# TAdeJong/pyGPA

Hardware: AMD Instinct MI355X
Metric: Mpixels/s displacement-field extraction (3 peaks, 4096^2 img) + achieved HBM GB/s (higher is better)
Workload: dtype f32; 1 GPU; 4096x4096 synthetic hex moire, 3 Bragg peaks x 16 k-vectors, sigma=10, weighted DCT-PCG unwrap kmax=10, image resident in HBM, u downloaded to pinned host memory inside the step (BASELINE.json configs[2]); x_planes=12, d2h_of_u=included, overlapped with the next step (copy stream), images_in_flight=1

## Files before the change

### pygpa_amd/csrc/gpa_api.hip

```cpp
#include "gpa_plan.h"

static thread_local std::string g_err;
int gpa_fail(int code, const std::string& msg) {
  g_err = msg;
  return code;
}
namespace gpa {
static const char* const kOptNames[OPT_COUNT] = {
    "PBS_FULLBAND", "SERIAL_UNWRAP", "NO_WORKER", "NO_KSPLIT", "NO_COMPACT", "NO_SHARED",
    "NO_PAIR", "TRI_SMALL", "TRI_Q", "NO_MR", "MR_FORCE_BLUESTEIN", "NO_ROWPQ", "COLSOLVE", "NO_LAT",
    "F32_EPS_FLOOR", "COLSTREAM_CHUNK", "NO_ROWHALF", "PAIR_MAXSIDE", "ROWHALF_MINLG", "NO_PQDCT",
    "NO_REORDER", "NO_RAW", "NO_TILEFUSE", "NO_ROWPERS", "NO_LFTILE", "LF_ALL_ROUNDS", "DFT_ENGINE", "GAUSS_FFT_MINR", "NO_GAUSS2D", "NO_DFT_HALF", "F32_STALL", "PBS_LDS_PAD", "NO_SHARED_PHASES", "PA_STAG", "PA_STAG_TICKS", "PA_ROT", "LF_STACK_BYTES", "NO_YSPEC"};
static OptVal g_opts[OPT_COUNT];
static std::once_flag g_opts_once;
static void opt_assign(OptVal& o, const char* value) {
  o.set = value != nullptr;
  o.num = value ? atof(value) : 0.0;
  memset(o.str, 0, sizeof(o.str));
  if (value) strncpy(o.str, value, sizeof(o.str) - 1);
}
static void opts_from_env() {
  for (int k = 0; k < OPT_COUNT; ++k) opt_assign(g_opts[k], getenv((std::string("GPA_") + kOptNames[k]).c_str()));
}
const OptVal& opt(OptKey k) {
  std::call_once(g_opts_once, opts_from_env);
  return g_opts[k];
}
}

Axis make_axis(int n) {
  Axis a;
  a.n = n;
  int lg = 0;
  while ((1 << lg) < n) ++lg;
  if ((1 << lg) == n) {
    a.padded = false;
  } else {
    lg = 0;
    while ((1 << lg) < 2 * n - 1) ++lg;
    a.padded = true;
  }
  if (lg < 6) {
    lg = 6;
    a.padded = ((1 << lg) != n);
  }
// ... 149 lines not shown
  p->serial_unwrap = opt_set(OPT_SERIAL_UNWRAP);
  p->use_worker = !opt_set(OPT_NO_WORKER);
  p->no_ksplit = opt_set(OPT_NO_KSPLIT);
  p->no_compact = opt_set(OPT_NO_COMPACT);
  p->use_shared = !opt_set(OPT_NO_SHARED);
  const int maxlg = dtype == GPA_F32 ? 14 : 13;
  if (n0 > 65536 || n1 > 65536) {
    fail(GPA_ERR_ARG, "gpa_plan_create: axis longer than 65536");
    delete p;
    return nullptr;
  }
  p->spectral_only = p->ax0.lg > maxlg || p->ax1.lg > maxlg;
  auto unwrap_axis_ok = [&](const Axis& a) { return a.lg <= maxlg || (a.lg == 14 && a.n == 16384); };
  p->no_unwrap = !(unwrap_axis_ok(p->ax0) && unwrap_axis_ok(p->ax1));
  if (plan_build(p) != GPA_OK) {
    std::string keep = g_err;
    gpa_plan_destroy(p);
    g_err = keep;
    return nullptr;
  }
  return p;
}

void gpa_plan_destroy(gpa_plan* p) {
  if (!p) return;
  hipSetDevice(p->device);
  delete p->worker;
  p->worker = nullptr;
  if (p->stream) hipStreamSynchronize(p->stream);
  void* bufs[] = {p->tw0, p->tw1, p->Hx, p->Hy, p->Tbuf, p->tb.cxb, p->tb.sx, p->tb.wxw, p->tb.wxr, p->tb.cyb, p->tb.sy, p->tb.wyw, p->tb.wyr, p->tb.planeof, p->d_pw,
                  p->tb.dx, p->tb.dy, p->d_kl, p->d_kr, p->d_image, p->d_mean, p->d_tile_mean, p->d_scratch,
                  p->d_lockin, p->d_kidx, p->d_dudx, p->d_dudy, p->d_wnorm, p->d_u, p->d_kmat, p->d_sf, p->d_grad, p->d_grads, p->d_absw, p->d_aux0, p->d_aux1,
                  p->sh.Gb, p->sh.psi, p->sh.dyc, p->sh.gtab, p->sh.desc, p->sh.order, p->d_taps, p->tw1s,
                  p->sh.pre, p->sh.rot16, p->d_wys, p->d_shifts, p->d_ystep, p->ys.Yhat, p->ys.strips, p->d_ys_pairs};
  for (void* b : bufs)
    if (b) hipFree(b);
  unwrap_workspace_destroy(&p->uw);
  unwrap_workspace_destroy(&p->uw2);
  if (p->uwb_images) unwrap_workspace_destroy(&p->uwb);
  if (p->have_uwp) unwrap_workspace_destroy(&p->uwp);
  if (p->d_wnorm_b) (void)hipFree(p->d_wnorm_b);
  if (p->h_iters_b) (void)hipHostFree(p->h_iters_b);
  for (void* b : {p->bT, p->bL, p->bMean, (void*)p->bScratch})
    if (b) (void)hipFree(b);
  if (p->stream2) { hipStreamSynchronize(p->stream2); hipStreamDestroy(p->stream2); }
  if (p->ev_fork) hipEventDestroy(p->ev_fork);
  if (p->ev_join) hipEventDestroy(p->ev_join);
  if (p->ev_x) hipEventDestroy(p->ev_x);
  if (p->d_tsum_part) (void)hipFree(p->d_tsum_part);
  warp_ws_free(&p->warp);
  ucell_ws_free(&p->ucell);
  dft_axis_destroy(&p->bx0);
  dft_axis_destroy(&p->bx1);
  dft_work_free(&p->dftw);
  for (auto& ax : p->gft)
    for (auto& g : ax) {
      if (g.H) (void)hipFree(g.H);
      if (g.tw) (void)hipFree(g.tw);
    }
  if (p->d_pertab) (void)hipFree(p->d_pertab);
  if (p->d_peakws) (void)hipFree(p->d_peakws);
  if (p->d_peaksmooth) (void)hipFree(p->d_peaksmooth);
  if (p->h_k) hipHostFree(p->h_k);
  if (p->h_iters) hipHostFree(p->h_iters);
  if (p->kprof) {
    for (int i = 0; i < p->kprof->npool; ++i) hipEventDestroy(p->kprof->pool[i]);
    delete p->kprof;
// ... 83 lines not shown
```

### pygpa_amd/csrc/gpa_api_tables.hip

```cpp
#include "gpa_plan.h"

void host_fft_pow2(std::vector<std::complex<double>>& a, bool inverse) {
  const size_t n = a.size();
  int lg = 0;
  while ((size_t(1) << lg) < n) ++lg;
  for (size_t i = 0; i < n; ++i) {
    size_t r = 0;
    for (int b = 0; b < lg; ++b) r |= ((i >> b) & 1) << (lg - 1 - b);
    if (r > i) std::swap(a[i], a[r]);
  }
  for (size_t len = 2; len <= n; len <<= 1) {
    const double ang = (inverse ? 2 : -2) * M_PI / (double)len;
    for (size_t s = 0; s < n; s += len)
      for (size_t j = 0; j < len / 2; ++j) {
        std::complex<double> w(cos(ang * (double)j), sin(ang * (double)j));
        auto u = a[s + j], v = a[s + j + len / 2] * w;
        a[s + j] = u + v;
        a[s + j + len / 2] = u - v;
      }
  }
}

std::vector<double> gaussian_kspace(int n, double sigma) {
  std::vector<double> g(n);
// ... 122 lines not shown
          const int Epad = (E + 15) & ~15;
          if (sa.L != cur.L && p->tw1s_L != sa.L) {
            if (!p->tw1s) TRY(dmalloc(p, &p->tw1s, (size_t)8192 * p->csz));
            TRY(upload_twiddles(p, p->tw1s, sa.L));
            p->tw1s_L = sa.L;
          }
          p->ax1s = sa;
          if (!p->d_taps) TRY(dmalloc(p, (void**)&p->d_taps, 1025 * sizeof(double)));
          if (!p->sh.gtab) TRY(dmalloc(p, &p->sh.gtab, (2 * 256 + 16) * p->rsz));
          HIP_TRY(hipMemcpyAsync(p->d_taps, taps.data(), ((size_t)mmax + 1) * sizeof(double), hipMemcpyHostToDevice, p->stream));
          HIP_TRY(hipStreamSynchronize(p->stream));
          std::vector<double> gt((size_t)2 * Epad + 16, 0.0);
          for (int m = 1; m <= E; ++m) gt[m] = taps[m];
          TRY(upload_real_table(p, p->sh.gtab, gt));
          p->sh_etab = mmax;
          p->sh_E = E;
          p->sh_Epad = Epad;
          p->sh_sigma = sigma;
          p->sh_ok = true;
        }
      }
    }
  }
  p->sigma_cached = sigma;
  return GPA_OK;
}

int shared_prepare(gpa_plan* p, int P, int K) {
  p->sh_use = false;
  p->ys_use = false;
  const int B = P * K;
  if (!p->sh_ok || !p->use_shared || K < 2 || (int)p->staged_planeof.size() < B) return GPA_OK;
  const bool reorder = !opt_set(OPT_NO_REORDER);
  if (p->sh_built_epoch == p->sh_epoch && p->sh_built_K == K && p->sh_built_B == B && p->sh_built_reorder == reorder) {
    p->sh_use = p->sh_built_ok;
    return GPA_OK;
  }
  p->sh_built_reorder = reorder;
  p->sh_built_epoch = -1;
  p->sh_built_ok = false;
  std::vector<int> order((size_t)B);
  for (int pp = 0; pp < P; ++pp) {
    bool aliased = false;
    for (int a = 0; a < K && !aliased; ++a)
      for (int b2 = a + 1; b2 < K && !aliased; ++b2) {
        const double *ka = &p->staged_kl[2 * ((size_t)pp * K + a)], *kb = &p->staged_kl[2 * ((size_t)pp * K + b2)];
        const bool same = ka[0] == kb[0] && ka[1] == kb[1];
        aliased = !same && ka[0] - floor(ka[0]) == kb[0] - floor(kb[0]) && ka[1] - floor(ka[1]) == kb[1] - floor(kb[1]);
      }
    std::vector<double> d2((size_t)K), pmin;
    std::vector<int> pfirst;
    int nplanes = 0;
    for (int k = 0; k < K; ++k) nplanes = std::max(nplanes, p->staged_planeof[pp * K + k] + 1);
    pmin.assign((size_t)nplanes, 1e300);
    pfirst.assign((size_t)nplanes, K);
    for (int k = 0; k < K; ++k) {
      const size_t b = (size_t)pp * K + k;
      const double ex = p->staged_kl[2 * b] - p->staged_kr[2 * b], ey = p->staged_kl[2 * b + 1] - p->staged_kr[2 * b + 1];
      d2[k] = ex * ex + ey * ey;
      const int pl = p->staged_planeof[b];
      pmin[pl] = std::min(pmin[pl], d2[k]);
      pfirst[pl] = std::min(pfirst[pl], k);
    }
    std::vector<int> idx((size_t)K);
    for (int k = 0; k < K; ++k) idx[k] = k;
    if (reorder && !aliased)
      std::stable_sort(idx.begin(), idx.end(), [&](int a, int b2) {
        const int pa = p->staged_planeof[pp * K + a], pb = p->staged_planeof[pp * K + b2];
        if (pa != pb) return pmin[pa] != pmin[pb] ? pmin[pa] < pmin[pb] : pfirst[pa] < pfirst[pb];
        return d2[a] < d2[b2];
      });
// ... 66 lines not shown
    p->sh_psi_bytes = ps;
  }
  if (!p->sh.rot16) TRY(dmalloc(p, &p->sh.rot16, (size_t)p->max_peaks * 16 * p->csz));
  if (!p->d_wys) TRY(dmalloc(p, (void**)&p->d_wys, (size_t)p->max_batch * sizeof(double)));
  if (!p->d_shifts) TRY(dmalloc(p, (void**)&p->d_shifts, (size_t)p->max_peaks * sizeof(int)));
  HIP_TRY(hipMemcpyAsync(p->d_wys, wys.data(), (size_t)B * sizeof(double), hipMemcpyHostToDevice, p->stream));
  HIP_TRY(hipMemcpyAsync(p->d_shifts, shifts.data(), (size_t)P * sizeof(int), hipMemcpyHostToDevice, p->stream));
  {
    std::vector<double> ys((size_t)P);
    p->sh_one_kref = true;
    for (int pp = 0; pp < P; ++pp) {
      const double c = p->staged_kr[2 * ((size_t)pp * K) + 1] + (double)shifts[pp] / EEs;
      ys[pp] = 2.0 * M_PI * (c - rint(c));
      for (int k = 1; k < K; ++k)
        if (p->staged_kr[2 * ((size_t)pp * K + k) + 1] != p->staged_kr[2 * ((size_t)pp * K) + 1]) p->sh_one_kref = false;
    }
    if (!p->d_ystep) TRY(dmalloc(p, (void**)&p->d_ystep, (size_t)p->max_peaks * sizeof(double)));
    HIP_TRY(hipMemcpyAsync(p->d_ystep, ys.data(), (size_t)P * sizeof(double), hipMemcpyHostToDevice, p->stream));
    HIP_TRY(hipStreamSynchronize(p->stream));
  }
  if (!p->sh.dyc) TRY(dmalloc(p, &p->sh.dyc, (size_t)p->max_peaks * p->n1 * p->csz));
  if (!p->sh.desc) TRY(dmalloc(p, (void**)&p->sh.desc, (size_t)p->max_batch * sizeof(int)));
  HIP_TRY(hipMemcpyAsync(p->sh.desc, desc.data(), (size_t)B * sizeof(int), hipMemcpyHostToDevice, p->stream));
  if (!p->sh.order) TRY(dmalloc(p, (void**)&p->sh.order, (size_t)p->max_batch * sizeof(int)));
  HIP_TRY(hipMemcpyAsync(p->sh.order, order.data(), (size_t)B * sizeof(int), hipMemcpyHostToDevice, p->stream));
  HIP_TRY(launch_shared_tables(p->dtype, p->ax1s, p->d_wys, p->d_kr, p->d_shifts, p->d_taps, p->sh_etab, p->sh_E, p->sh_Epad, B, K,
                               p->sh_nbl, p->sh, p->stream));
  HIP_TRY(hipStreamSynchronize(p->stream));
  p->ys_ok = false;
  if (passB_yspec_supports(p->dtype, p->ax1s, p->sh_nbl) && p->ax1s.L == p->ax1.L && !p->ax1.padded) {
    const int nplanes = p->last_planes;
    std::vector<unsigned> mask((size_t)nplanes, 0u);
    for (int b = 0; b < B; ++b) mask[p->staged_planeof[b]] |= yspec_blockmask(p->ax1s.lg, shifts[b / K], p->sh_nbl);
    std::vector<int> pairs;
    unsigned all = 0;
    for (int slot = 0; slot < 16; ++slot)
      for (int q = 0; q < nplanes; ++q) {
        int seen = 0;
        for (int blk = 0; blk < 16; ++blk)
          if ((mask[q] >> blk) & 1) {
            if (seen++ == slot) pairs.push_back(q | (blk << 16));
          }
        all |= mask[q];
      }
    if (!p->d_ys_pairs) TRY(dmalloc(p, (void**)&p->d_ys_pairs, (size_t)p->max_batch * 16 * sizeof(int)));
    HIP_TRY(hipMemcpyAsync(p->d_ys_pairs, pairs.data(), pairs.size() * sizeof(int), hipMemcpyHostToDevice, p->stream));
    HIP_TRY(hipStreamSynchronize(p->stream));
    p->ys.pairs = p->d_ys_pairs;
    p->ys.npairs = (int)pairs.size();
    p->ys.blockmask = all;
    p->ys.E = p->sh_E;
    p->ys.Epad = p->sh_Epad;
    p->ys_ok = !pairs.empty();
  }
  p->sh_built_epoch = p->sh_epoch;
  p->sh_built_K = K;
  p->sh_built_B = B;
  p->sh_built_ok = true;
  p->sh_use = true;
  return GPA_OK;
}

int stage_kvectors(gpa_plan* p, const double* kl, const double* kr_per_b, int B, int* planes_out) {
  p->ys_use = false;
  if ((int)p->staged_kl.size() == 2 * B && memcmp(p->staged_kl.data(), kl, (size_t)B * 2 * sizeof(double)) == 0 &&
      memcmp(p->staged_kr.data(), kr_per_b, (size_t)B * 2 * sizeof(double)) == 0) {
    *planes_out = p->last_planes;
    return GPA_OK;
  }
  HIP_TRY(hipStreamSynchronize(p->stream));
  p->staged_kl.assign(kl, kl + 2 * (size_t)B);
  p->staged_kr.assign(kr_per_b, kr_per_b + 2 * (size_t)B);
  double* h_kl = p->h_k;
  double* h_kr = p->h_k + 2 * (size_t)B;
  double* h_pw = p->h_k + 4 * (size_t)B;
  int* h_po = reinterpret_cast<int*>(p->h_k + 5 * (size_t)B);
  memcpy(h_kl, kl, (size_t)B * 2 * sizeof(double));
  memcpy(h_kr, kr_per_b, (size_t)B * 2 * sizeof(double));
  int Bx = 0;
  for (int b = 0; b < B; ++b) {
    int found = -1;
    for (int q = 0; q < Bx; ++q)
      if (memcmp(&h_pw[q], &kl[2 * b], sizeof(double)) == 0) { found = q; break; }
    if (found < 0) { h_pw[Bx] = kl[2 * b]; found = Bx++; }
    h_po[b] = found;
  }
// ... 70 lines not shown
```

### pygpa_amd/csrc/gpa_internal.h

```cpp
#pragma once
#include <hip/hip_runtime.h>
#include <stdint.h>

#include "gpa_fft.h"
#include "gpa_mrfft.h"

#ifndef GPA_F64_WAVES
#define GPA_F64_WAVES 2
#endif

namespace gpa {

struct KernelProfiler {
  struct Rec { const char* name; hipEvent_t a, b; };
  static constexpr int MAXREC = 4096;
  Rec rec[MAXREC];
  int n = 0;
  hipEvent_t pool[2 * MAXREC];
  int npool = 0;
};
extern thread_local KernelProfiler* g_kprof;
struct ProfScope {
  hipStream_t s;
  KernelProfiler::Rec* r = nullptr;
// ... 15 lines not shown
__device__ __forceinline__ int xcd_tile(int b, int grid) {
  const int base = grid >> 3, rem = grid & 7, x = b & 7, idx = b >> 3;
  return x * base + (x < rem ? x : rem) + idx;
}
#endif

inline hipError_t set_dynamic_lds_once(const void* kern, int bytes, unsigned& done) {
  int dev = 0;
  (void)hipGetDevice(&dev);
  const unsigned bit = 1u << (dev & 31);
  if (done & bit) return hipSuccess;
  hipError_t e = hipFuncSetAttribute(kern, hipFuncAttributeMaxDynamicSharedMemorySize, bytes);
  if (e == hipSuccess) done |= bit;
  return e;
}

inline int device_cus() {
  static int n[32] = {};
  int dev = 0;
  (void)hipGetDevice(&dev);
  int& slot = n[dev & 31];
  if (!slot) {
    int cus = 0;
    if (hipDeviceGetAttribute(&cus, hipDeviceAttributeMultiprocessorCount, dev) != hipSuccess || cus <= 0) cus = 256;
    slot = cus;
  }
  return slot;
}

enum OptKey {
  OPT_PBS_FULLBAND, OPT_SERIAL_UNWRAP, OPT_NO_WORKER, OPT_NO_KSPLIT, OPT_NO_COMPACT, OPT_NO_SHARED,
  OPT_NO_PAIR, OPT_TRI_SMALL, OPT_TRI_Q, OPT_NO_MR, OPT_MR_FORCE_BLUESTEIN, OPT_NO_ROWPQ,
  OPT_COLSOLVE, OPT_NO_LAT, OPT_F32_EPS_FLOOR, OPT_COLSTREAM_CHUNK, OPT_NO_ROWHALF, OPT_PAIR_MAXSIDE, OPT_ROWHALF_MINLG, OPT_NO_PQDCT,
  OPT_NO_REORDER, OPT_NO_RAW, OPT_NO_TILEFUSE, OPT_NO_ROWPERS, OPT_NO_LFTILE, OPT_LF_ALL_ROUNDS, OPT_DFT_ENGINE, OPT_GAUSS_FFT_MINR, OPT_NO_GAUSS2D, OPT_NO_DFT_HALF, OPT_F32_STALL, OPT_PBS_LDS_PAD, OPT_NO_SHARED_PHASES, OPT_PA_STAG, OPT_PA_STAG_TICKS, OPT_PA_ROT, OPT_LF_STACK_BYTES, OPT_NO_YSPEC, OPT_COUNT
};
struct OptVal {
  bool set;
  double num;
  char str[24];
};
const OptVal& opt(OptKey k);
inline bool opt_set(OptKey k) { return opt(k).set; }

#define GPA_PROF_CAT2(a, b) a##b
#define GPA_PROF_CAT(a, b) GPA_PROF_CAT2(a, b)
#define GPA_PROF(name, stream) ::gpa::ProfScope GPA_PROF_CAT(_gpa_prof_, __LINE__)(name, stream)

struct Axis {
  int n;
  int lg;
  int L;
  bool padded;
  int extL, extR;
};
inline int axis_tpf(const Axis& a) { return a.L / 16; }

GPA_HD int axis_src(int m, int n, int L, bool padded, int extL, int extR) {
  if (!padded) return m;
  if (m < n) return m;
  if (m < n + extR) return m - n;
  if (m >= L - extL) return m - L + n;
  return -1;
}

struct SweepTables {
  void* cxb;
  void* sx;
  void* wxw;
  void* wxr;
  void* cyb;
  void* sy;
  void* wyw;
  void* wyr;
  void* dx;
  void* dy;
  int* planeof;
};

hipError_t launch_tables(int dtype, const Axis& a0, const Axis& a1, const double* kl,
                         const double* kr, int B, const double* pw, int Bx, const SweepTables& tb,
                         hipStream_t s);
hipError_t launch_mean(int dtype, const void* image, size_t count, double* scratch,
                       void* mean_out, hipStream_t s, int nimg = 1);
hipError_t launch_passA(int dtype, const Axis& a0, int n1, const void* image, const void* mean,
                        const SweepTables& tb, const void* Hx, const void* tw0, void* Tbuf,
                        int Bx, hipStream_t s, int nimg = 1);
struct PassAYspec {
  void* Yhat;
  void* strips;
  const int* pairs;
  int npairs;
  unsigned blockmask;
  int E, Epad;
};
hipError_t launch_passA_yspec(int dtype, const Axis& a0, const Axis& a1, const void* image, const void* mean,
                              const SweepTables& tb, const void* Hx, const void* tw0, const void* tw1, void* Tbuf, int Bx,
                              const PassAYspec& ys, hipStream_t s, int nimg = 1);
hipError_t launch_passB(int dtype, const Axis& a1, int n0, const void* Tbuf, const void* Hy,
                        const void* tw1, const SweepTables& tb, int P, int K, bool select,
                        void* out, int32_t* kidx, hipStream_t s, int nimg = 1, int Bx = 0);
hipError_t launch_passB_ext(int dtype, const Axis& a1, int n0, const void* Tbuf, const void* Hy, const void* tw1,
                            const SweepTables& tb, int K, int mode, void* out, int32_t* kidx, const uint8_t* gate,
                            void* psi, hipStream_t s, int P = 1);
hipError_t launch_passB_split(int dtype, const Axis& a1, int n0, const void* Tbuf, const void* Hy, const void* tw1,
                              const SweepTables& tb, int P, int K, int ksplit, void* part, int32_t* pidx, void* out,
                              int32_t* kidx, hipStream_t s);
hipError_t launch_phasegrad(int dtype, const void* psi, int K, const int32_t* kidx, int n0, int n1, const double* kl,
                            const double* kr, int mode, void* grad, hipStream_t s, const double* ystep = nullptr, int P = 1);
int passA_cols(int dtype, int lg);
int spec_index_rt(int lg, int tid, int reg, int elems = 16);

hipError_t launch_reconstruct(int dtype, const void* lockin, const double* kmat ,
                              int P, int n0, int n1, int border, void* dudx, void* dudy,
                              void* wnorm, hipStream_t s, const double* ystep = nullptr );

hipError_t launch_reconstruct_tile(int dtype, const void* lockin, const double* kmat, int P, int n0, int n1, int border,
                                   int i0, int j0, int t0, int t1, void* const dx[2], size_t dx_pitch, void* const dy[2],
                                   size_t dy_pitch, void* const wn[2], size_t wn_pitch, hipStream_t s,
                                   const double* ystep = nullptr);
hipError_t launch_reconstruct_setup(int dtype, const void* lockin, const double* kmat, int P, int n0, int n1,
                                    int border, void* wnorm, void* r0, void* r1, double* part0, double* part1,
                                    int* nparts, hipStream_t s, int nimg = 1, size_t rstride = 0, size_t pstride = 0,
                                    const double* ystep = nullptr );

// ... 81 lines not shown
```

### pygpa_amd/csrc/gpa_plan.h

```cpp
#pragma once
#include <math.h>
#include <stdio.h>
#include <stdlib.h>
#include <string.h>

#include <algorithm>
#include <complex>
#include <condition_variable>
#include <functional>
#include <mutex>
#include <thread>
#include <string>
#include <limits>
#include <vector>

#include "../../include/gpa_hip.h"
#include "gpa_internal.h"
#include "gpa_passb_shared.h"
#include "gpa_yspec.h"
#include "gpa_unwrap.h"
#include "gpa_dft.h"
#include "gpa_gaussfft.h"

using namespace gpa;
// ... 82 lines not shown
  Axis ax0{}, ax1{};
  Axis ax0_full{}, ax1_full{};
  hipStream_t stream = nullptr;
  size_t rsz = 4, csz = 8;
  size_t ws_bytes = 0;
  void* tw0 = nullptr;
  void* tw1 = nullptr;
  void* Hx = nullptr;
  void* Hy = nullptr;
  double sigma_cached = -1.0;
  PassBSharedTables sh{};
  double* d_taps = nullptr;
  int sh_etab = 0, sh_E = 0, sh_Epad = 0;
  int sh_nbl = 16;
  double sh_sigma = 0.0;
  double* d_wys = nullptr;
  int* d_shifts = nullptr;
  Axis ax1s{};
  void* tw1s = nullptr;
  int tw1s_L = 0;
  bool sh_ok = false;
  bool use_shared = true;
  int sh_epoch = 0, sh_built_epoch = -1, sh_built_K = 0, sh_built_B = 0;
  bool sh_built_reorder = true;
  double* d_ystep = nullptr;
  bool sh_one_kref = true;
  bool lk_raw = false;
  bool sh_built_ok = false;
  bool sh_use = false;
  size_t sh_gb_bytes = 0, sh_psi_bytes = 0;
  bool ys_ok = false;
  bool ys_use = false;
  PassAYspec ys{};
  int* d_ys_pairs = nullptr;
  size_t ys_yhat_bytes = 0, ys_strips_bytes = 0;
  std::vector<int> staged_planeof;
  void* Tbuf = nullptr;
  int tbuf_planes = 0;
  SweepTables tb{};
  double* d_kl = nullptr;
  double* d_kr = nullptr;
  double* d_pw = nullptr;
  int last_planes = 0;
  std::vector<double> staged_kl, staged_kr, staged_kmat;
  int* h_iters = nullptr;
  int iters_stride = 1;
  int iters_off = 0;
  UnwrapWorkspace uwp{};
  bool have_uwp = false, use_pair = false;
  double* h_k = nullptr;
  void* d_image = nullptr;
  void* d_mean = nullptr;
  void* d_tile_mean = nullptr;
  double* d_tsum_part = nullptr;
  size_t tsum_cap = 0;
  hipEvent_t ev_x = nullptr;
  double tile_mean = std::numeric_limits<double>::quiet_NaN();
  void* d_sf = nullptr;
  size_t sf_bytes = 0;
  void* d_grad = nullptr;
  void* d_grads = nullptr;
  void* d_absw = nullptr;
  double* d_scratch = nullptr;
  void* d_aux0 = nullptr;
  void* d_aux1 = nullptr;
  void* d_lockin = nullptr;
  int32_t* d_kidx = nullptr;
// ... 118 lines not shown
```

### pygpa_amd/csrc/gpa_sweep.hip

```cpp
#include "gpa_internal.h"
#include "gpa_passb.h"
#include "gpa_yspec.h"

namespace gpa {

thread_local KernelProfiler* g_kprof = nullptr;

template <class T>
__device__ __forceinline__ cpx<T> unit_phasor(double cycles) {
  double fr = cycles - rint(cycles);
  double s, c;
  sincospi(2.0 * fr, &s, &c);
  return {(T)c, (T)s};
}

template <class T>
__global__ void tables_kernel(const double* __restrict__ kl, const double* __restrict__ kr,
                              const double* __restrict__ pw, int B, int Bx, int n0, int n1, int L0, int L1, int tpf0, int tpf1,
                              cpx<T>* cxb, cpx<T>* sx, cpx<T>* wxw, cpx<T>* wxr, cpx<T>* cyb, cpx<T>* sy, cpx<T>* wyw,
                              cpx<T>* wyr,
                              cpx<T>* dx, cpx<T>* dy) {
  const int b = blockIdx.y;
  const int j = blockIdx.x * blockDim.x + threadIdx.x;
  if (b < Bx) {
// ... 112 lines not shown
#ifndef GPA_PA_C10
#define GPA_PA_C10 8
#endif
#ifndef GPA_PA_C9
#define GPA_PA_C9 16
#endif
#ifndef GPA_PA_C11
#define GPA_PA_C11 4
#endif
#ifndef GPA_PA_C12
#define GPA_PA_C12 16
#endif
    int c = LG == 10 ? GPA_PA_C10 : (LG == 9 ? GPA_PA_C9 : (LG == 11 ? GPA_PA_C11 : (LG == 12 ? GPA_PA_C12 : 16)));
    while (c > 1 && (c * F::TPF > 1024 || (size_t)c * (F::LDS_ELEMS + 32) * sizeof(cpx<T>) > 160 * 1024)) c /= 2;
    return c;
  }
  static constexpr int C = cols();
  static constexpr int NT = (sizeof(T) == 4 && C >= 2) ? 2 : 1;
  static constexpr int CT = C / NT;
  static constexpr int REGION = CT * F::LDS_ELEMS;
  static constexpr int THREADS = CT * F::TPF;
  static constexpr size_t LDS_BYTES = (size_t)NT * REGION * sizeof(cpx<T>);
  static constexpr bool FITS = (size_t)(F::LDS_ELEMS + 32) * sizeof(cpx<T>) <= 160 * 1024;
};

enum { PA_SPATIAL = 0, PA_YSPEC = 1, PA_STRIPS = 2 };
template <class T, int LG, bool PADDED, int MODE = PA_SPATIAL>
__global__ __launch_bounds__((PassAGeom<T, LG>::THREADS)) void passA_kernel(
    const T* __restrict__ image, const T* __restrict__ mean, int n0, int n1,
    const cpx<T>* __restrict__ cxb, const cpx<T>* __restrict__ sx, const cpx<T>* __restrict__ wxw,
    const cpx<T>* __restrict__ wxr, int extL, int extR,
    const typename HType<PADDED, T>::type* __restrict__ H,
    const cpx<T>* __restrict__ twtab, cpx<T>* __restrict__ Tout, int B, int bchunk, int stag_phases, int stag_ticks,
    int stag_first, int rot_mul, const cpx<T>* __restrict__ Yin, const int* __restrict__ pairs, int npairs, int ntl,
    int opitch) {
  using F = WgFFT<T, LG>;
  using G = PassAGeom<T, LG>;
  constexpr int CT = G::CT, NT = G::NT, TPF = F::TPF, L = F::L;
  extern __shared__ __attribute__((aligned(16))) char smem[];
  const int c = threadIdx.x % CT, t = threadIdx.x / CT;
  cpx<T>* lds = reinterpret_cast<cpx<T>*>(smem) + c;
  constexpr int LDS_NSTRIDE = G::REGION;
  int tile = xcd_tile(blockIdx.x, gridDim.x);
  if (MODE == PA_SPATIAL && stag_phases < 0) {
    constexpr int TPL0 = (128 / (int)(G::C * sizeof(cpx<T>))) > 0 ? (128 / (int)(G::C * sizeof(cpx<T>))) : 1;
    const int g = TPL0 * -stag_phases, x = blockIdx.x & 7, idx = blockIdx.x >> 3;
    if (gridDim.x % (8 * g) == 0) tile = ((idx / g) * 8 + x) * g + idx % g;
  }
  int y0 = tile * G::C + c * NT;
  int oy0 = y0;
  int plane = 0;
  const int op = MODE == PA_STRIPS ? opitch : n1;
  if constexpr (MODE == PA_YSPEC) {
    constexpr int TPL = (128 / (int)(G::C * sizeof(cpx<T>))) > 0 ? (128 / (int)(G::C * sizeof(cpx<T>))) : 1;
    const int tl = tile % TPL, pr = (tile / TPL) % npairs, ln = tile / (TPL * npairs);
    const int pe = pairs[pr];
    plane = pe & 0xffff;
    y0 = (pe >> 16) * (n1 >> 4) + (ln * TPL + tl) * G::C + c * NT;
    oy0 = y0;
  } else if constexpr (MODE == PA_STRIPS) {
    y0 = (tile < ntl ? tile * G::C : n1 - (2 * ntl - tile) * G::C) + c * NT;
    oy0 = tile < ntl ? y0 : y0 - (n1 - opitch);
  }
  if constexpr (MODE == PA_YSPEC) Yin += (size_t)blockIdx.z * n0 * n1;
  else image += (size_t)blockIdx.z * n0 * n1;
  Tout += (size_t)blockIdx.z * B * n0 * op;
  const T m = (MODE != PA_YSPEC && mean) ? mean[blockIdx.z] : T(0);

  T val[MODE == PA_YSPEC ? 1 : NT][16];
  cpx<T> cval[MODE == PA_YSPEC ? NT : 1][16];
  unsigned wrapmask = 0, rightmask = 0;
#pragma unroll
  for (int i = 0; i < 16; ++i) {
    const int slot = t + TPF * i;
    const int xs = axis_src(slot, n0, L, PADDED, extL, extR);
    if (PADDED && slot >= n0) { if (slot < n0 + extR) rightmask |= 1u << i; else wrapmask |= 1u << i; }
    if constexpr (MODE == PA_YSPEC) {
      struct alignas(NT * sizeof(cpx<T>)) Cols { cpx<T> v[NT]; };
      Cols cc;
#pragma unroll
      for (int n = 0; n < NT; ++n) cc.v[n] = {T(0), T(0)};
      if (xs >= 0) cc = *reinterpret_cast<const Cols*>(&Yin[(size_t)xs * n1 + y0]);
#pragma unroll
      for (int n = 0; n < NT; ++n) cval[n][i] = cc.v[n];
    } else {
#pragma unroll
      for (int n = 0; n < NT; ++n) {
        const int y = y0 + n;
        val[n][i] = (y < n1 && xs >= 0) ? image[(size_t)xs * n1 + y] - m : T(0);
      }
    }
  }
  typename F::KTw tw;
  F::load_twiddles(tw, twtab, t);
  if (MODE == PA_SPATIAL && stag_phases > 1 && (int)blockIdx.x < stag_first) {
    constexpr int TPL = (128 / (int)(G::C * sizeof(cpx<T>))) > 0 ? (128 / (int)(G::C * sizeof(cpx<T>))) : 1;
    const int ph = (tile / TPL) % stag_phases;
    asm volatile("s_waitcnt vmcnt(0)" ::: "memory");
    if (ph) {
      const unsigned long long t0 = wall_clock64(), wait = (unsigned long long)ph * (unsigned)stag_ticks;
      while (wall_clock64() - t0 < wait) __builtin_amdgcn_s_sleep(4);
    }
    __syncthreads();
  }

  const int b0 = MODE == PA_YSPEC ? plane : blockIdx.y * bchunk;
  const int b1 = MODE == PA_YSPEC ? plane + 1 : ((b0 + bchunk < B) ? b0 + bchunk : B);
  const int nb = b1 - b0;
  int b = b0 + (nb > 0 ? (int)(((unsigned)(tile * G::C * (int)sizeof(cpx<T>) / 128) * (unsigned)rot_mul) % (unsigned)nb) : 0);
  for (int j = 0; j < nb; ++j, b = (b + 1 < b1 ? b + 1 : b0)) {
    F::refresh(tw);
    const cpx<T> base = cxb[(size_t)b * TPF + t];
    cpx<T> x[NT][16];
#pragma unroll
    for (int i = 0; i < 16; ++i) {
      cpx<T> ph = cmul(base, sx[b * 16 + i]);
      if (PADDED && ((wrapmask >> i) & 1)) ph = cmul(ph, wxw[b]);
      if (PADDED && ((rightmask >> i) & 1)) ph = cmul(ph, wxr[b]);
#pragma unroll
      for (int n = 0; n < NT; ++n) {
        if constexpr (MODE == PA_YSPEC) x[n][i] = cmul(cval[n][i], ph);
        else x[n][i] = {val[n][i] * ph.x, val[n][i] * ph.y};
      }
    }
    F::template forward_multi<NT, CT>(x, lds, LDS_NSTRIDE, t, tw);
    {
      const typename HType<PADDED, T>::type* Hb = H;
      asm volatile("" : "+s"(Hb));
#pragma unroll
      for (int i = 0; i < 16; ++i) {
        const auto h = hload<PADDED, T>(Hb, i * TPF + t);
#pragma unroll
        for (int n = 0; n < NT; ++n) x[n][i] = hmul(x[n][i], h);
      }
    }
    F::template inverse_multi<NT, CT>(x, lds, LDS_NSTRIDE, t, tw);
    bool paired = false;
    if constexpr (NT == 2) {
      if (y0 + 1 < n1 && (op & 1) == 0) {
        paired = true;
        struct alignas(2 * sizeof(cpx<T>)) Pair { cpx<T> a, b; };
        auto put = [&](int i) {
          const int slot = t + TPF * i;
          if (!PADDED || slot < n0) {
            Pair pr = {x[0][i], x[1][i]};
            *reinterpret_cast<Pair*>(&Tout[((size_t)b * n0 + slot) * op + oy0]) = pr;
          }
        };
#pragma unroll
        for (int i = 0; i < 16; ++i) put(i);
      }
    }
    if (!paired) {
#pragma unroll
      for (int n = 0; n < NT; ++n) {
        const int y = y0 + n;
        if (y < n1) {
#pragma unroll
          for (int i = 0; i < 16; ++i) {
            const int slot = t + TPF * i;
            if (!PADDED || slot < n0) Tout[((size_t)b * n0 + slot) * op + oy0 + n] = x[n][i];
          }
        }
      }
    }
  }
}

template <class T, int LG, bool PADDED, int MODE>
static hipError_t run_passA(const Axis& a0, int n1, const void* image, const void* mean,
                            const SweepTables& tb, const void* Hx, const void* tw0, void* Tbuf,
                            int B, hipStream_t s, int nimg, const PassAYspec* ys) {
  using G = PassAGeom<T, LG>;
  if constexpr (!G::FITS) {
    return hipErrorInvalidValue;
  } else {
    auto kern = passA_kernel<T, LG, PADDED, MODE>;
    static unsigned lds_set = 0;
    hipError_t e = set_dynamic_lds_once(reinterpret_cast<const void*>(kern), (int)G::LDS_BYTES, lds_set);
    if (e != hipSuccess) return e;
    int tiles = (n1 + G::C - 1) / G::C, ntl = 0, opitch = n1;
    if (MODE == PA_YSPEC) {
      if (n1 % (16 * G::C) || ((size_t)(n1 / 16) * sizeof(cpx<T>)) % 128 || ys->npairs < 1) return hipErrorInvalidValue;
      tiles = ys->npairs * (n1 / 16 / G::C);
    } else if (MODE == PA_STRIPS) {
      ntl = (ys->E + G::C - 1) / G::C;
      opitch = 2 * ys->Epad;
      if (n1 % G::C || ntl * G::C > ys->Epad || 2 * ntl * G::C > n1) return hipErrorInvalidValue;
      tiles = 2 * ntl;
    }
    int ysplit = 1;
    while (MODE != PA_YSPEC && tiles * ysplit < 512 && ysplit < B) ysplit *= 2;
    if (ysplit > B) ysplit = B;
    const int bchunk = (B + ysplit - 1) / ysplit;
    dim3 grid(tiles, (B + bchunk - 1) / bchunk, nimg);
    const int stag = opt_set(OPT_PA_STAG) ? (int)opt(OPT_PA_STAG).num : 0;
    const int stag_ticks = opt_set(OPT_PA_STAG_TICKS) ? (int)opt(OPT_PA_STAG_TICKS).num : 800 / (stag > 1 ? stag : 1);
    GPA_PROF(MODE == PA_STRIPS ? "passA_strips_kernel" : "passA_kernel", s);
    kern<<<grid, G::THREADS, G::LDS_BYTES, s>>>(
        (const T*)image, (const T*)mean, a0.n, n1, (const cpx<T>*)tb.cxb, (const cpx<T>*)tb.sx,
        (const cpx<T>*)tb.wxw, (const cpx<T>*)tb.wxr, a0.extL, a0.extR,
        (const typename HType<PADDED, T>::type*)Hx, (const cpx<T>*)tw0, (cpx<T>*)(MODE == PA_STRIPS ? ys->strips : Tbuf), B, bchunk, stag,
        stag_ticks, device_cus(), opt_set(OPT_PA_ROT) ? (int)opt(OPT_PA_ROT).num : (LG >= 12 ? 1 : 0),
        (const cpx<T>*)(ys ? ys->Yhat : nullptr), ys ? ys->pairs : nullptr, ys ? ys->npairs : 0, ntl, opitch);
    return hipGetLastError();
  }
}

template <int MODE>
static hipError_t dispatch_passA(int dtype, const Axis& a0, int n1, const void* image, const void* mean,
                                 const SweepTables& tb, const void* Hx, const void* tw0, void* Tbuf,
                                 int B, hipStream_t s, int nimg, const PassAYspec* ys) {
#define CASE_A(LG)                                                                                \
  case LG:                                                                                        \
    if (dtype == 0)                                                                               \
      return a0.padded ? run_passA<float, LG, true, MODE>(a0, n1, image, mean, tb, Hx, tw0, Tbuf, B, s, nimg, ys) \
                       : run_passA<float, LG, false, MODE>(a0, n1, image, mean, tb, Hx, tw0, Tbuf, B, s, nimg, ys); \
    else                                                                                          \
      return a0.padded ? run_passA<double, LG, true, MODE>(a0, n1, image, mean, tb, Hx, tw0, Tbuf, B, s, nimg, ys) \
                       : run_passA<double, LG, false, MODE>(a0, n1, image, mean, tb, Hx, tw0, Tbuf, B, s, nimg, ys);
  switch (a0.lg) { GPA_FOR_LG(CASE_A) }
#undef CASE_A
  return hipErrorInvalidValue;
}

hipError_t launch_passA(int dtype, const Axis& a0, int n1, const void* image, const void* mean,
                        const SweepTables& tb, const void* Hx, const void* tw0, void* Tbuf,
                        int B, hipStream_t s, int nimg) {
  return dispatch_passA<PA_SPATIAL>(dtype, a0, n1, image, mean, tb, Hx, tw0, Tbuf, B, s, nimg, nullptr);
}

template <class T, int LG>
__global__ __launch_bounds__((WgFFT<T, LG, 16>::TPF)) void rowfft_kernel(const T* __restrict__ image, const T* __restrict__ mean,
                                                                        int n0, const cpx<T>* __restrict__ twtab,
                                                                        unsigned blockmask, cpx<T>* __restrict__ Yhat) {
  using F = WgFFT<T, LG, 16>;
  constexpr int TPF = F::TPF, L = F::L;
// ... 84 lines not shown
```

### pygpa_amd/csrc/gpa_yspec.h

```cpp
#pragma once
#include "gpa_fft.h"

namespace gpa {

GPA_HD bool yspec_lg_ok(int lg) { return lg == 11 || lg == 12; }

struct YspecSrc { int tid, reg; };

GPA_HD YspecSrc yspec_source(int lg, int s, int tid, int reg) {
  const int odd = lg == 11 ? (s & 1) : 0;
  YspecSrc r;
  r.tid = odd ? (tid ^ 8) : tid;
  r.reg = (reg + s - odd + ((odd && (tid & 8)) ? 2 : 0)) & 15;
  return r;
}

GPA_HD unsigned yspec_blockmask(int lg, int s, int nbl) {
  unsigned m = 0;
  for (int i = 0; i < nbl; ++i) {
    m |= 1u << yspec_source(lg, s, 0, i).reg;
    m |= 1u << yspec_source(lg, s, 8, i).reg;
  }
  return m;
}

}
```

Before: 3377 Mpixels/s.

## Group yspec passA planes per block so one loaded tile serves several planes

The yspec pass-A mode now groups the planes that share a y-block (up to a configurable group size, default 6 for f32) instead of launching one workgroup per (plane, block) pair. Each workgroup loads its Yhat column tile once, keeps it in registers, and loops over the group's planes, which cuts redundant reads of Yhat from HBM. The block index is also remapped with an 8-way interleave and a per-group rotation to spread memory traffic. In exchange there are fewer workgroups, higher register pressure from keeping the tile, and stricter size-divisibility checks.

```diff
diff --git a/pygpa_amd/csrc/gpa_api.hip b/pygpa_amd/csrc/gpa_api.hip
--- a/pygpa_amd/csrc/gpa_api.hip
+++ b/pygpa_amd/csrc/gpa_api.hip
@@ -10,7 +10,7 @@
     "PBS_FULLBAND", "SERIAL_UNWRAP", "NO_WORKER", "NO_KSPLIT", "NO_COMPACT", "NO_SHARED",
     "NO_PAIR", "TRI_SMALL", "TRI_Q", "NO_MR", "MR_FORCE_BLUESTEIN", "NO_ROWPQ", "COLSOLVE", "NO_LAT",
     "F32_EPS_FLOOR", "COLSTREAM_CHUNK", "NO_ROWHALF", "PAIR_MAXSIDE", "ROWHALF_MINLG", "NO_PQDCT",
-    "NO_REORDER", "NO_RAW", "NO_TILEFUSE", "NO_ROWPERS", "NO_LFTILE", "LF_ALL_ROUNDS", "DFT_ENGINE", "GAUSS_FFT_MINR", "NO_GAUSS2D", "NO_DFT_HALF", "F32_STALL", "PBS_LDS_PAD", "NO_SHARED_PHASES", "PA_STAG", "PA_STAG_TICKS", "PA_ROT", "LF_STACK_BYTES", "NO_YSPEC"};
+    "NO_REORDER", "NO_RAW", "NO_TILEFUSE", "NO_ROWPERS", "NO_LFTILE", "LF_ALL_ROUNDS", "DFT_ENGINE", "GAUSS_FFT_MINR", "NO_GAUSS2D", "NO_DFT_HALF", "F32_STALL", "PBS_LDS_PAD", "NO_SHARED_PHASES", "PA_STAG", "PA_STAG_TICKS", "PA_ROT", "LF_STACK_BYTES", "NO_YSPEC", "YSPEC_GROUP"};
 static OptVal g_opts[OPT_COUNT];
 static std::once_flag g_opts_once;
 static void opt_assign(OptVal& o, const char* value) {
@@ -226,7 +226,7 @@
                   p->tb.dx, p->tb.dy, p->d_kl, p->d_kr, p->d_image, p->d_mean, p->d_tile_mean, p->d_scratch,
                   p->d_lockin, p->d_kidx, p->d_dudx, p->d_dudy, p->d_wnorm, p->d_u, p->d_kmat, p->d_sf, p->d_grad, p->d_grads, p->d_absw, p->d_aux0, p->d_aux1,
                   p->sh.Gb, p->sh.psi, p->sh.dyc, p->sh.gtab, p->sh.desc, p->sh.order, p->d_taps, p->tw1s,
-                  p->sh.pre, p->sh.rot16, p->d_wys, p->d_shifts, p->d_ystep, p->ys.Yhat, p->ys.strips, p->d_ys_pairs};
+                  p->sh.pre, p->sh.rot16, p->d_wys, p->d_shifts, p->d_ystep, p->ys.Yhat, p->ys.strips, p->d_ys_groups};
   for (void* b : bufs)
     if (b) hipFree(b);
   unwrap_workspace_destroy(&p->uw);
diff --git a/pygpa_amd/csrc/gpa_api_tables.hip b/pygpa_amd/csrc/gpa_api_tables.hip
--- a/pygpa_amd/csrc/gpa_api_tables.hip
+++ b/pygpa_amd/csrc/gpa_api_tables.hip
@@ -178,11 +178,14 @@
   const int B = P * K;
   if (!p->sh_ok || !p->use_shared || K < 2 || (int)p->staged_planeof.size() < B) return GPA_OK;
   const bool reorder = !opt_set(OPT_NO_REORDER);
-  if (p->sh_built_epoch == p->sh_epoch && p->sh_built_K == K && p->sh_built_B == B && p->sh_built_reorder == reorder) {
+  const int gmax = opt_set(OPT_YSPEC_GROUP) ? std::max(1, (int)opt(OPT_YSPEC_GROUP).num) : yspec_group_default(p->dtype);
+  if (p->sh_built_epoch == p->sh_epoch && p->sh_built_K == K && p->sh_built_B == B && p->sh_built_reorder == reorder &&
+      p->ys_gmax == gmax) {
     p->sh_use = p->sh_built_ok;
     return GPA_OK;
   }
   p->sh_built_reorder = reorder;
+  p->ys_gmax = gmax;
   p->sh_built_epoch = -1;
   p->sh_built_ok = false;
   std::vector<int> order((size_t)B);
@@ -315,26 +318,24 @@
     const int nplanes = p->last_planes;
     std::vector<unsigned> mask((size_t)nplanes, 0u);
     for (int b = 0; b < B; ++b) mask[p->staged_planeof[b]] |= yspec_blockmask(p->ax1s.lg, shifts[b / K], p->sh_nbl);
-    std::vector<int> pairs;
     unsigned all = 0;
-    for (int slot = 0; slot < 16; ++slot)
-      for (int q = 0; q < nplanes; ++q) {
-        int seen = 0;
-        for (int blk = 0; blk < 16; ++blk)
-          if ((mask[q] >> blk) & 1) {
-            if (seen++ == slot) pairs.push_back(q | (blk << 16));
-          }
-        all |= mask[q];
-      }
-    if (!p->d_ys_pairs) TRY(dmalloc(p, (void**)&p->d_ys_pairs, (size_t)p->max_batch * 16 * sizeof(int)));
-    HIP_TRY(hipMemcpyAsync(p->d_ys_pairs, pairs.data(), pairs.size() * sizeof(int), hipMemcpyHostToDevice, p->stream));
+    for (int q = 0; q < nplanes; ++q) all |= mask[q];
+    const YspecGroups yg = yspec_groups(mask.data(), nplanes, gmax);
+    const size_t cap = (size_t)p->max_batch * 16;
+    if (yg.planes.size() > cap) return GPA_ERR_STATE;
+    std::vector<int> stage(yg.planes);
+    stage.resize(cap, 0);
+    for (const YspecGroup& g : yg.groups) { stage.push_back(g.block); stage.push_back(g.first); stage.push_back(g.count); }
+    if (!p->d_ys_groups) TRY(dmalloc(p, (void**)&p->d_ys_groups, cap * 4 * sizeof(int)));
+    HIP_TRY(hipMemcpyAsync(p->d_ys_groups, stage.data(), stage.size() * sizeof(int), hipMemcpyHostToDevice, p->stream));
     HIP_TRY(hipStreamSynchronize(p->stream));
-    p->ys.pairs = p->d_ys_pairs;
-    p->ys.npairs = (int)pairs.size();
+    p->ys.planes = p->d_ys_groups;
+    p->ys.groups = p->d_ys_groups + cap;
+    p->ys.ngroups = (int)yg.groups.size();
     p->ys.blockmask = all;
     p->ys.E = p->sh_E;
     p->ys.Epad = p->sh_Epad;
-    p->ys_ok = !pairs.empty();
+    p->ys_ok = !yg.groups.empty();
   }
   p->sh_built_epoch = p->sh_epoch;
   p->sh_built_K = K;
diff --git a/pygpa_amd/csrc/gpa_internal.h b/pygpa_amd/csrc/gpa_internal.h
--- a/pygpa_amd/csrc/gpa_internal.h
+++ b/pygpa_amd/csrc/gpa_internal.h
@@ -71,7 +71,7 @@
   OPT_PBS_FULLBAND, OPT_SERIAL_UNWRAP, OPT_NO_WORKER, OPT_NO_KSPLIT, OPT_NO_COMPACT, OPT_NO_SHARED,
   OPT_NO_PAIR, OPT_TRI_SMALL, OPT_TRI_Q, OPT_NO_MR, OPT_MR_FORCE_BLUESTEIN, OPT_NO_ROWPQ,
   OPT_COLSOLVE, OPT_NO_LAT, OPT_F32_EPS_FLOOR, OPT_COLSTREAM_CHUNK, OPT_NO_ROWHALF, OPT_PAIR_MAXSIDE, OPT_ROWHALF_MINLG, OPT_NO_PQDCT,
-  OPT_NO_REORDER, OPT_NO_RAW, OPT_NO_TILEFUSE, OPT_NO_ROWPERS, OPT_NO_LFTILE, OPT_LF_ALL_ROUNDS, OPT_DFT_ENGINE, OPT_GAUSS_FFT_MINR, OPT_NO_GAUSS2D, OPT_NO_DFT_HALF, OPT_F32_STALL, OPT_PBS_LDS_PAD, OPT_NO_SHARED_PHASES, OPT_PA_STAG, OPT_PA_STAG_TICKS, OPT_PA_ROT, OPT_LF_STACK_BYTES, OPT_NO_YSPEC, OPT_COUNT
+  OPT_NO_REORDER, OPT_NO_RAW, OPT_NO_TILEFUSE, OPT_NO_ROWPERS, OPT_NO_LFTILE, OPT_LF_ALL_ROUNDS, OPT_DFT_ENGINE, OPT_GAUSS_FFT_MINR, OPT_NO_GAUSS2D, OPT_NO_DFT_HALF, OPT_F32_STALL, OPT_PBS_LDS_PAD, OPT_NO_SHARED_PHASES, OPT_PA_STAG, OPT_PA_STAG_TICKS, OPT_PA_ROT, OPT_LF_STACK_BYTES, OPT_NO_YSPEC, OPT_YSPEC_GROUP, OPT_COUNT
 };
 struct OptVal {
   bool set;
@@ -127,8 +127,9 @@
 struct PassAYspec {
   void* Yhat;
   void* strips;
-  const int* pairs;
-  int npairs;
+  const int* groups;
+  const int* planes;
+  int ngroups;
   unsigned blockmask;
   int E, Epad;
 };
diff --git a/pygpa_amd/csrc/gpa_plan.h b/pygpa_amd/csrc/gpa_plan.h
--- a/pygpa_amd/csrc/gpa_plan.h
+++ b/pygpa_amd/csrc/gpa_plan.h
@@ -138,7 +138,8 @@
   bool ys_ok = false;
   bool ys_use = false;
   PassAYspec ys{};
-  int* d_ys_pairs = nullptr;
+  int* d_ys_groups = nullptr;
+  int ys_gmax = 0;
   size_t ys_yhat_bytes = 0, ys_strips_bytes = 0;
   std::vector<int> staged_planeof;
   void* Tbuf = nullptr;
diff --git a/pygpa_amd/csrc/gpa_sweep.hip b/pygpa_amd/csrc/gpa_sweep.hip
--- a/pygpa_amd/csrc/gpa_sweep.hip
+++ b/pygpa_amd/csrc/gpa_sweep.hip
@@ -168,8 +168,8 @@
     const cpx<T>* __restrict__ wxr, int extL, int extR,
     const typename HType<PADDED, T>::type* __restrict__ H,
     const cpx<T>* __restrict__ twtab, cpx<T>* __restrict__ Tout, int B, int bchunk, int stag_phases, int stag_ticks,
-    int stag_first, int rot_mul, const cpx<T>* __restrict__ Yin, const int* __restrict__ pairs, int npairs, int ntl,
-    int opitch) {
+    int stag_first, int rot_mul, const cpx<T>* __restrict__ Yin, const int* __restrict__ groups,
+    const int* __restrict__ gplanes, int ntl, int opitch) {
   using F = WgFFT<T, LG>;
   using G = PassAGeom<T, LG>;
   constexpr int CT = G::CT, NT = G::NT, TPF = F::TPF, L = F::L;
@@ -185,14 +185,17 @@
   }
   int y0 = tile * G::C + c * NT;
   int oy0 = y0;
-  int plane = 0;
+  int gfirst = 0, gcount = 0, grot = 0;
   const int op = MODE == PA_STRIPS ? opitch : n1;
   if constexpr (MODE == PA_YSPEC) {
     constexpr int TPL = (128 / (int)(G::C * sizeof(cpx<T>))) > 0 ? (128 / (int)(G::C * sizeof(cpx<T>))) : 1;
-    const int tl = tile % TPL, pr = (tile / TPL) % npairs, ln = tile / (TPL * npairs);
-    const int pe = pairs[pr];
-    plane = pe & 0xffff;
-    y0 = (pe >> 16) * (n1 >> 4) + (ln * TPL + tl) * G::C + c * NT;
+    const int lpx = (n1 >> 7) / (G::C * TPL);
+    const int x = blockIdx.x & 7, idx = blockIdx.x >> 3;
+    const int tl = idx % TPL, ln = x * lpx + (idx / TPL) % lpx, g = idx / (TPL * lpx);
+    gfirst = groups[3 * g + 1];
+    gcount = groups[3 * g + 2];
+    grot = ln + g;
+    y0 = groups[3 * g] * (n1 >> 4) + (ln * TPL + tl) * G::C + c * NT;
     oy0 = y0;
   } else if constexpr (MODE == PA_STRIPS) {
     y0 = (tile < ntl ? tile * G::C : n1 - (2 * ntl - tile) * G::C) + c * NT;
@@ -206,20 +209,29 @@
   T val[MODE == PA_YSPEC ? 1 : NT][16];
   cpx<T> cval[MODE == PA_YSPEC ? NT : 1][16];
   unsigned wrapmask = 0, rightmask = 0;
+  constexpr bool KEEP = MODE == PA_YSPEC && !PADDED && G::THREADS <= 512;
+  const unsigned toff = (unsigned)t * (unsigned)n1 + (unsigned)y0;
+  auto load_tile = [&](unsigned off, int yc) {
+    struct alignas(NT * sizeof(cpx<T>)) Cols { cpx<T> v[NT]; };
+#pragma unroll
+    for (int i = 0; i < 16; ++i) {
+      const int xs = axis_src(t + TPF * i, n0, L, PADDED, extL, extR);
+      Cols cc;
+#pragma unroll
+      for (int n = 0; n < NT; ++n) cc.v[n] = {T(0), T(0)};
+      if constexpr (!PADDED) cc = *reinterpret_cast<const Cols*>(Yin + (size_t)(TPF * i) * n1 + off);
+      else if (xs >= 0) cc = *reinterpret_cast<const Cols*>(&Yin[(size_t)xs * n1 + yc]);
+#pragma unroll
+      for (int n = 0; n < (MODE == PA_YSPEC ? NT : 1); ++n) cval[n][i] = cc.v[n];
+    }
+  };
+  if constexpr (KEEP) load_tile(toff, y0);
 #pragma unroll
   for (int i = 0; i < 16; ++i) {
     const int slot = t + TPF * i;
     const int xs = axis_src(slot, n0, L, PADDED, extL, extR);
     if (PADDED && slot >= n0) { if (slot < n0 + extR) rightmask |= 1u << i; else wrapmask |= 1u << i; }
-    if constexpr (MODE == PA_YSPEC) {
-      struct alignas(NT * sizeof(cpx<T>)) Cols { cpx<T> v[NT]; };
-      Cols cc;
-#pragma unroll
-      for (int n = 0; n < NT; ++n) cc.v[n] = {T(0), T(0)};
-      if (xs >= 0) cc = *reinterpret_cast<const Cols*>(&Yin[(size_t)xs * n1 + y0]);
-#pragma unroll
-      for (int n = 0; n < NT; ++n) cval[n][i] = cc.v[n];
-    } else {
+    if constexpr (MODE != PA_YSPEC) {
 #pragma unroll
       for (int n = 0; n < NT; ++n) {
         const int y = y0 + n;
@@ -240,11 +252,19 @@
     __syncthreads();
   }
 
-  const int b0 = MODE == PA_YSPEC ? plane : blockIdx.y * bchunk;
-  const int b1 = MODE == PA_YSPEC ? plane + 1 : ((b0 + bchunk < B) ? b0 + bchunk : B);
+  const int b0 = MODE == PA_YSPEC ? 0 : blockIdx.y * bchunk;
+  const int b1 = MODE == PA_YSPEC ? gcount : ((b0 + bchunk < B) ? b0 + bchunk : B);
   const int nb = b1 - b0;
-  int b = b0 + (nb > 0 ? (int)(((unsigned)(tile * G::C * (int)sizeof(cpx<T>) / 128) * (unsigned)rot_mul) % (unsigned)nb) : 0);
-  for (int j = 0; j < nb; ++j, b = (b + 1 < b1 ? b + 1 : b0)) {
+  const int rq = MODE == PA_YSPEC ? grot : tile * G::C * (int)sizeof(cpx<T>) / 128;
+  int bb = b0 + (nb > 0 ? (int)(((unsigned)rq * (unsigned)rot_mul) % (unsigned)nb) : 0);
+  for (int j = 0; j < nb; ++j, bb = (bb + 1 < b1 ? bb + 1 : b0)) {
+    const int b = MODE == PA_YSPEC ? gplanes[gfirst + bb] : bb;
+    if constexpr (MODE == PA_YSPEC && !KEEP) {
+      unsigned o = toff;
+      int yc = y0;
+      asm volatile("" : "+v"(o), "+v"(yc));
+      load_tile(o, yc);
+    }
     F::refresh(tw);
     const cpx<T> base = cxb[(size_t)b * TPF + t];
     cpx<T> x[NT][16];
@@ -280,7 +300,8 @@
           const int slot = t + TPF * i;
           if (!PADDED || slot < n0) {
             Pair pr = {x[0][i], x[1][i]};
-            *reinterpret_cast<Pair*>(&Tout[((size_t)b * n0 + slot) * op + oy0]) = pr;
+            if constexpr (MODE == PA_YSPEC && !PADDED) *reinterpret_cast<Pair*>(Tout + ((size_t)b * n0 + TPF * i) * n1 + toff) = pr;
+            else *reinterpret_cast<Pair*>(&Tout[((size_t)b * n0 + slot) * op + oy0]) = pr;
           }
         };
 #pragma unroll
@@ -295,7 +316,8 @@
 #pragma unroll
           for (int i = 0; i < 16; ++i) {
             const int slot = t + TPF * i;
-            if (!PADDED || slot < n0) Tout[((size_t)b * n0 + slot) * op + oy0 + n] = x[n][i];
+            if constexpr (MODE == PA_YSPEC && !PADDED) Tout[((size_t)b * n0 + TPF * i) * n1 + toff + n] = x[n][i];
+            else if (!PADDED || slot < n0) Tout[((size_t)b * n0 + slot) * op + oy0 + n] = x[n][i];
           }
         }
       }
@@ -317,8 +339,9 @@
     if (e != hipSuccess) return e;
     int tiles = (n1 + G::C - 1) / G::C, ntl = 0, opitch = n1;
     if (MODE == PA_YSPEC) {
-      if (n1 % (16 * G::C) || ((size_t)(n1 / 16) * sizeof(cpx<T>)) % 128 || ys->npairs < 1) return hipErrorInvalidValue;
-      tiles = ys->npairs * (n1 / 16 / G::C);
+      constexpr int TPL = (128 / (int)(G::C * sizeof(cpx<T>))) > 0 ? (128 / (int)(G::C * sizeof(cpx<T>))) : 1;
+      if (n1 % (128 * G::C * TPL) || ((size_t)(n1 / 16) * sizeof(cpx<T>)) % 128 || ys->ngroups < 1) return hipErrorInvalidValue;
+      tiles = ys->ngroups * (n1 / 16 / G::C);
     } else if (MODE == PA_STRIPS) {
       ntl = (ys->E + G::C - 1) / G::C;
       opitch = 2 * ys->Epad;
@@ -338,7 +361,7 @@
         (const cpx<T>*)tb.wxw, (const cpx<T>*)tb.wxr, a0.extL, a0.extR,
         (const typename HType<PADDED, T>::type*)Hx, (const cpx<T>*)tw0, (cpx<T>*)(MODE == PA_STRIPS ? ys->strips : Tbuf), B, bchunk, stag,
         stag_ticks, device_cus(), opt_set(OPT_PA_ROT) ? (int)opt(OPT_PA_ROT).num : (LG >= 12 ? 1 : 0),
-        (const cpx<T>*)(ys ? ys->Yhat : nullptr), ys ? ys->pairs : nullptr, ys ? ys->npairs : 0, ntl, opitch);
+        (const cpx<T>*)(ys ? ys->Yhat : nullptr), ys ? ys->groups : nullptr, ys ? ys->planes : nullptr, ntl, opitch);
     return hipGetLastError();
   }
 }
diff --git a/pygpa_amd/csrc/gpa_yspec.h b/pygpa_amd/csrc/gpa_yspec.h
--- a/pygpa_amd/csrc/gpa_yspec.h
+++ b/pygpa_amd/csrc/gpa_yspec.h
@@ -1,4 +1,7 @@
 #pragma once
+#include <algorithm>
+#include <vector>
+
 #include "gpa_fft.h"
 
 namespace gpa {
@@ -24,4 +27,29 @@
   return m;
 }
 
+struct YspecGroup { int block, first, count; };
+struct YspecGroups {
+  std::vector<YspecGroup> groups;
+  std::vector<int> planes;
+};
+
+inline YspecGroups yspec_groups(const unsigned* mask, int nplanes, int gmax) {
+  YspecGroups r;
+  if (gmax < 1) gmax = 1;
+  for (int blk = 0; blk < 16; ++blk) {
+    int run = 0;
+    for (int q = 0; q < nplanes; ++q) {
+      if (!((mask[q] >> blk) & 1)) continue;
+      if (run == 0 || run == gmax) { r.groups.push_back({blk, (int)r.planes.size(), 0}); run = 0; }
+      r.planes.push_back(q);
+      ++r.groups.back().count;
+      ++run;
+    }
+  }
+  std::stable_sort(r.groups.begin(), r.groups.end(), [](const YspecGroup& a, const YspecGroup& b) { return a.count > b.count; });
+  return r;
 }
+
+inline int yspec_group_default(int dtype) { return dtype == 0 ? 6 : 12; }
+
+}
```

Measured after the change: 3597 Mpixels/s (median of 6 runs). +6.5%, better.
